# reilabs/gnark-whir

Hardware: AMD Instinct MI355X
Metric: Groth16 proofs/sec for WHIR-verifier circuit (2^20 poly); G1 MSM pts/sec (higher is better)
Workload: dtype u32x8 Montgomery (BN254 Fr/Fp, exact modular integers)

## Files before the change

### gnark-whir_amd/csrc/ntt.hip

```cpp
#include "ctx.h"
#include "ntt_wave.cuh"
#include "msm2_core.cuh"
#include <cstring>
#include <cstdlib>

struct NttState {
    u32 log_n = 0xffffffffu;
    Fr *small_f = nullptr, *small_i = nullptr, *tw64k_f = nullptr, *tw64k_i = nullptr;
    Fr *tw_lo_f = nullptr, *tw_hi_f = nullptr, *tw_lo_i = nullptr, *tw_hi_i = nullptr;
    Fr *g_lo = nullptr, *g_hi = nullptr, *gi_lo = nullptr, *gi_hi = nullptr, *ninv = nullptr;
    Fr *g_hi_n = nullptr, *gi_hi_nd = nullptr;
    Fr *ninv_den = nullptr;
    u32 tw_h = 0;
    Fr *d_tw_inv = nullptr, *d_tw_fwd = nullptr, *d_sc_fwd = nullptr, *d_sc_inv = nullptr;
    u32 d_log_n = 0xffffffffu, d_log_r0 = 0, d_npass = 0;
    u32 direct_min_log_n = 12;
    u32 log_e = 9, max_contig = 9, max_strided = 7, threads = 256;
    u32 lds_floor = 0;
    u32 plan_set = 0;
    u32 wave_stages = 1;
    u32 fuse_pair = 1;
    u32 fuse_triple = 1;
    u32 fuse_last = 1;
};
static NttKnobs knobs_for(const struct NttState *st, u32 log_n);
static NttState *state_of(mi_ctx *ctx) {
    static_assert(sizeof(NttState) <= 384, "NttState lives in ctx->ntt_state");
    return reinterpret_cast<NttState *>(ctx->ntt_state);
}

template <int CC> __global__ void k_ntt_contig_last_sub_count(Fr *A, const Fr *Cin, NttPass pa, NttTables ta, NttPass pc, NttTables tc, Msm2Shape zs, u32 *C1);
typedef void (*LastSubCountKernel)(Fr *, const Fr *, NttPass, NttTables, NttPass, NttTables, Msm2Shape, u32 *);
static const LastSubCountKernel k_last_sub_count[6] = {
    k_ntt_contig_last_sub_count<17>, k_ntt_contig_last_sub_count<18>, k_ntt_contig_last_sub_count<19>,
    k_ntt_contig_last_sub_count<20>, k_ntt_contig_last_sub_count<21>, k_ntt_contig_last_sub_count<22>};
bool mi_ntt_set_knob(mi_ctx *ctx, const char *name, int64_t value) {
    if (!std::strcmp(name, "ntt_lds_floor_kb") && value >= 0 && value <= 160) { state_of(ctx)->lds_floor = (u32)value * 1024u; return true; }
    return false;
}
void mi_ntt_state_free(mi_ctx *ctx) {
    NttState *st = state_of(ctx);
    Fr **all[] = {&st->small_f, &st->small_i, &st->tw64k_f, &st->tw64k_i, &st->g_hi_n, &st->gi_hi_nd, &st->tw_lo_f, &st->tw_hi_f, &st->tw_lo_i, &st->tw_hi_i,
                  &st->g_lo, &st->g_hi, &st->gi_lo, &st->gi_hi, &st->ninv, &st->ninv_den, &st->d_tw_inv, &st->d_tw_fwd, &st->d_sc_fwd, &st->d_sc_inv};
    for (Fr **p : all) if (*p) { (void)hipFree(*p); *p = nullptr; }
}

void mi_ntt_state_trim(mi_ctx *ctx) {
    mi_ntt_state_free(ctx);
    NttState *st = state_of(ctx);
    st->log_n = 0xffffffffu; st->d_log_n = 0xffffffffu; st->d_log_r0 = 0; st->d_npass = 0;
}
size_t mi_ntt_table_bytes(mi_ctx *ctx) {
    const NttState *st = state_of(ctx);
    size_t b = 0;
    if (st->small_f) b += (size_t)(2 * 2048 + 2 * 65536) * sizeof(Fr);
    if (st->log_n != 0xffffffffu) {
        const size_t nlo = (size_t)1 << st->tw_h, nhi = (size_t)1 << (st->log_n - st->tw_h);
        b += (4 * nlo + 6 * nhi + 2) * sizeof(Fr);
    }
    for (const Fr *p : {st->d_tw_inv, st->d_tw_fwd, st->d_sc_fwd, st->d_sc_inv}) if (p) b += sizeof(Fr) << st->d_log_n;
    return b;
}

static NttKnobs knobs_for(const NttState *st, u32 log_n) {
    if (st->plan_set) return NttKnobs{st->log_e, st->max_contig, st->max_strided};
    if (log_n == 24) return NttKnobs{10, 8, 8};
    if (log_n >= 25) return NttKnobs{10, 10, 8};
    return NttKnobs{st->log_e, st->max_contig, st->max_strided};
}

__global__ void k_pow_table(Fr *out, u32 count, Fr base, Fr c, u32 shift) {
    u32 j = blockIdx.x * blockDim.x + threadIdx.x;
    if (j >= count) return;
    u64 e = (u64)j << shift;
    Fr acc = c, b = base;
    while (e) {
        if (e & 1) acc = acc * b;
        b = fe_sqr(b);
        e >>= 1;
    }
    out[j] = acc;
}

__global__ void __launch_bounds__(1024) k_ntt_pass(Fr *dst, const Fr *src, NttPass p, NttTables t) {
    extern __shared__ U4 lds[];
    const u64 tile = blockIdx.x;
    ntt_tile_load(p, t, src, tile, threadIdx.x, blockDim.x, lds);
    __syncthreads();
    for (u32 s = 0; s < p.log_r; s++) {
        ntt_tile_stage(p, t, s, threadIdx.x, blockDim.x, lds);
        __syncthreads();
    }
    ntt_tile_store(p, t, dst, tile, threadIdx.x, blockDim.x, lds);
}

#ifndef MI_NTT_WAVES_PER_EU
#define MI_NTT_WAVES_PER_EU 1
#endif
__global__ void __launch_bounds__(256, MI_NTT_WAVES_PER_EU) k_ntt_pass_wave(Fr *dst, const Fr *src, NttPass p, NttTables t) {
    extern __shared__ U4 lds[];
    const u64 tile = blockIdx.x;
    const u32 PL = ntt_plane_slots(p);
    ntt_tile_load(p, t, src, tile, threadIdx.x, blockDim.x, lds);
    __syncthreads();
    if (!p.dit)
        for (u32 s = 0; s + 7 < p.log_r; s++) {
            ntt_tile_stage(p, t, s, threadIdx.x, blockDim.x, lds);
            __syncthreads();
        }
    const u32 lane = threadIdx.x & 63, wave = threadIdx.x >> 6, nwaves = blockDim.x >> 6;
    const u32 nsub = 1u << (p.log_r + p.log_c - 7);
    for (u32 sb = wave; sb < nsub; sb += nwaves) {
        const u32 col = sb & ((1u << p.log_c) - 1), base = (sb >> p.log_c) << 7;
        u32 ra, rb, wa, wb;
        if (!p.dit) { ra = base + lane; rb = ra + 64; wa = base + 2 * lane; wb = wa + 1; }
        else { ra = base + 2 * lane; rb = ra + 1; wa = base + lane; wb = wa + 64; }
        Fr x0 = lds_get(lds, PL, ntt_lds_slot(p, ra, col)), x1 = lds_get(lds, PL, ntt_lds_slot(p, rb, col));
        wave_ntt128(x0, x1, lane, p.dit != 0, t.small);
        lds_put(lds, PL, ntt_lds_slot(p, wa, col), x0);
        lds_put(lds, PL, ntt_lds_slot(p, wb, col), x1);
    }
    __syncthreads();
    if (p.dit)
        for (u32 s = 7; s < p.log_r; s++) {
            ntt_tile_stage(p, t, s, threadIdx.x, blockDim.x, lds);
            __syncthreads();
        }
    ntt_tile_store(p, t, dst, tile, threadIdx.x, blockDim.x, lds);
}

__global__ void __launch_bounds__(256) k_ntt_contig_pair(Fr *data, NttPass pi, NttTables ti, NttPass pf, NttTables tf) {
    extern __shared__ U4 lds[];
    const u64 tile = blockIdx.x;
    const u32 PL = ntt_plane_slots(pi);
    ntt_tile_load(pi, ti, data, tile, threadIdx.x, blockDim.x, lds);
    __syncthreads();
    for (u32 s = 0; s + 7 < pi.log_r; s++) {
        ntt_tile_stage(pi, ti, s, threadIdx.x, blockDim.x, lds);
        __syncthreads();
    }
    const u32 lane = threadIdx.x & 63, wave = threadIdx.x >> 6, nwaves = blockDim.x >> 6;
    const u32 nsub = 1u << (pi.log_r + pi.log_c - 7);
    for (u32 sb = wave; sb < nsub; sb += nwaves) {
        const u32 col = sb & ((1u << pi.log_c) - 1), base = (sb >> pi.log_c) << 7;
        Fr x0 = lds_get(lds, PL, ntt_lds_slot(pi, base + lane, col)), x1 = lds_get(lds, PL, ntt_lds_slot(pi, base + lane + 64, col));
        wave_ntt128(x0, x1, lane, false, ti.small);
        const u32 r0 = base + 2 * lane, r1 = r0 + 1;
        Fr f;
        if (ntt_edge_factor(pi, ti, r0, ntt_global_index(pi, tile, r0, col), 1, f)) x0 = fe_mul_lazy(x0, f);
        if (ntt_edge_factor(pf, tf, r0, ntt_global_index(pf, tile, r0, col), 0, f)) x0 = fe_mul_lazy(x0, f);
        if (ntt_edge_factor(pi, ti, r1, ntt_global_index(pi, tile, r1, col), 1, f)) x1 = fe_mul_lazy(x1, f);
        if (ntt_edge_factor(pf, tf, r1, ntt_global_index(pf, tile, r1, col), 0, f)) x1 = fe_mul_lazy(x1, f);
        wave_ntt128(x0, x1, lane, true, tf.small);
        lds_put(lds, PL, ntt_lds_slot(pf, base + lane, col), x0);
        lds_put(lds, PL, ntt_lds_slot(pf, base + lane + 64, col), x1);
    }
    __syncthreads();
    for (u32 s = 7; s < pf.log_r; s++) {
        ntt_tile_stage(pf, tf, s, threadIdx.x, blockDim.x, lds);
        __syncthreads();
    }
    ntt_tile_store(pf, tf, data, tile, threadIdx.x, blockDim.x, lds);
}

__global__ void __launch_bounds__(512) k_ntt_strided_triple(Fr *a, const Fr *b, NttPass pc, NttTables tc, NttPass pl, NttTables tl) {
    extern __shared__ U4 lds[];
    const u64 tile = blockIdx.x;
    const u32 PL = ntt_plane_slots(pc);
    const u32 lane = threadIdx.x & 63, sb = threadIdx.x >> 6;
    const u32 col = sb & ((1u << pc.log_c) - 1), base = (sb >> pc.log_c) << 7;
    const u32 s0 = ntt_lds_slot(pc, base + 2 * lane, col), s1 = ntt_lds_slot(pc, base + 2 * lane + 1, col);
    ntt_tile_load(pc, tc, a, tile, threadIdx.x, blockDim.x, lds);
    __syncthreads();
    Fr a0 = lds_get(lds, PL, s0), a1 = lds_get(lds, PL, s1);
    wave_ntt128(a0, a1, lane, true, tc.small);
    __syncthreads();
    ntt_tile_load(pc, tc, b, tile, threadIdx.x, blockDim.x, lds);
    __syncthreads();
    Fr x0 = lds_get(lds, PL, s0), x1 = lds_get(lds, PL, s1);
    wave_ntt128(x0, x1, lane, true, tc.small);
    x0 = ntt_mul_lazy2(x0, a0); x1 = ntt_mul_lazy2(x1, a1);
    wave_ntt128(x0, x1, lane, false, tl.small);
    __syncthreads();
    lds_put(lds, PL, ntt_lds_slot(pl, base + 2 * lane, col), x0);
    lds_put(lds, PL, ntt_lds_slot(pl, base + 2 * lane + 1, col), x1);
    __syncthreads();
    ntt_tile_store(pl, tl, a, tile, threadIdx.x, blockDim.x, lds);
}
__global__ void __launch_bounds__(256) k_ntt_strided_triple8(Fr *a, const Fr *b, NttPass pc, NttTables tc, NttPass pl, NttTables tl) {
    extern __shared__ U4 lds[];
    const u64 tile = blockIdx.x;
    const u32 PL = ntt_plane_slots(pc);
    const u32 lane = threadIdx.x & 63, wave = threadIdx.x >> 6, nwaves = blockDim.x >> 6;
    const u32 C = 1u << pc.log_c, nsub = 2u << pc.log_c;
    const u32 nb = C >> 1;
    Fr keep[4];
    auto reg_stages = [&](const NttPass &p, bool dit, const Fr *small) {
        for (u32 sbk = wave; sbk < nsub; sbk += nwaves) {
            const u32 col = sbk & (C - 1), base = (sbk >> p.log_c) << 7;
            u32 ra, rb, wa, wb;
            if (!dit) { ra = base + lane; rb = ra + 64; wa = base + 2 * lane; wb = wa + 1; }
            else { ra = base + 2 * lane; rb = ra + 1; wa = base + lane; wb = wa + 64; }
            Fr x0 = lds_get(lds, PL, ntt_lds_slot(p, ra, col)), x1 = lds_get(lds, PL, ntt_lds_slot(p, rb, col));
            wave_ntt128(x0, x1, lane, dit, small);
            lds_put(lds, PL, ntt_lds_slot(p, wa, col), x0);
            lds_put(lds, PL, ntt_lds_slot(p, wb, col), x1);
        }
    };
    ntt_tile_load(pc, tc, a, tile, threadIdx.x, blockDim.x, lds);
    __syncthreads();
    reg_stages(pc, true, tc.small);
    __syncthreads();
#pragma unroll
    for (u32 k = 0; k < 2; k++) {
        if (k >= nb) break;
        const u32 bf = threadIdx.x + 256 * k, col = bf & (C - 1), j = bf >> pc.log_c;
        Fr x = lds_get(lds, PL, ntt_lds_slot(pc, j, col));
        Fr y = lds_get(lds, PL, ntt_lds_slot(pc, j + 128, col));
        ntt_bfly_dit(x, y, j ? &tc.small[j << 4] : nullptr);
        keep[2 * k] = x; keep[2 * k + 1] = y;
    }
    __syncthreads();
    ntt_tile_load(pc, tc, b, tile, threadIdx.x, blockDim.x, lds);
    __syncthreads();
    reg_stages(pc, true, tc.small);
    __syncthreads();
#pragma unroll
    for (u32 k = 0; k < 2; k++) {
        if (k >= nb) break;
        const u32 bf = threadIdx.x + 256 * k, col = bf & (C - 1), j = bf >> pc.log_c;
        Fr x = lds_get(lds, PL, ntt_lds_slot(pc, j, col));
        Fr y = lds_get(lds, PL, ntt_lds_slot(pc, j + 128, col));
        ntt_bfly_dit(x, y, j ? &tc.small[j << 4] : nullptr);
        Fr p0 = ntt_mul_lazy2(x, keep[2 * k]), p1 = ntt_mul_lazy2(y, keep[2 * k + 1]);
        ntt_bfly_dif(p0, p1, j ? &tl.small[j << 4] : nullptr);
        lds_put(lds, PL, ntt_lds_slot(pl, j, col), p0);
        lds_put(lds, PL, ntt_lds_slot(pl, j + 128, col), p1);
    }
    __syncthreads();
    reg_stages(pl, false, tl.small);
    __syncthreads();
    ntt_tile_store(pl, tl, a, tile, threadIdx.x, blockDim.x, lds);
}

__device__ __forceinline__ void ntt_wave_pass_to_lds(const NttPass &p, const NttTables &t, const Fr *src, u64 tile, U4 *lds) {
    const u32 PL = ntt_plane_slots(p);
    ntt_tile_load(p, t, src, tile, threadIdx.x, blockDim.x, lds);
    __syncthreads();
    for (u32 s = 0; s + 7 < p.log_r; s++) {
        ntt_tile_stage(p, t, s, threadIdx.x, blockDim.x, lds);
        __syncthreads();
    }
    const u32 lane = threadIdx.x & 63, wave = threadIdx.x >> 6, nwaves = blockDim.x >> 6;
    const u32 nsub = 1u << (p.log_r + p.log_c - 7);
    for (u32 sb = wave; sb < nsub; sb += nwaves) {
        const u32 col = sb & ((1u << p.log_c) - 1), base = (sb >> p.log_c) << 7;
        Fr x0 = lds_get(lds, PL, ntt_lds_slot(p, base + lane, col)), x1 = lds_get(lds, PL, ntt_lds_slot(p, base + lane + 64, col));
        wave_ntt128(x0, x1, lane, false, t.small);
        lds_put(lds, PL, ntt_lds_slot(p, base + 2 * lane, col), x0);
        lds_put(lds, PL, ntt_lds_slot(p, base + 2 * lane + 1, col), x1);
    }
    __syncthreads();
}
template <int CC>
__device__ __forceinline__ void ntt_contig_last_sub_body(Fr *A, const Fr *Cin, const NttPass &pa, const NttTables &ta, const NttPass &pc, const NttTables &tc,
                                                         const Msm2Shape &zs, u32 *C1) {
    extern __shared__ U4 lds[];
    const u64 tile = blockIdx.x;
    const u32 E = 1u << (pa.log_r + pa.log_c), PL = ntt_plane_slots(pa);
    u32 *cnt = reinterpret_cast<u32 *>(lds + 2 * PL);
    const u32 nsl = E / MSM2_SLICE;
    if (CC >= 0) for (u32 k = threadIdx.x; k < nsl * zs.ngroups; k += blockDim.x) cnt[k] = 0;
    Fr keep[4];
    ntt_wave_pass_to_lds(pc, tc, Cin, tile, lds);
#pragma unroll
    for (u32 k = 0; k < 4; k++) {
        const u32 e = threadIdx.x + k * blockDim.x;
        if (e >= E) break;
        const u32 rho = e & ((1u << pc.log_r) - 1), col = e >> pc.log_r;
        Fr v = lds_get(lds, PL, ntt_lds_slot(pc, rho, col)), f;
        if (ntt_edge_factor(pc, tc, rho, ntt_global_index(pc, tile, rho, col), 1, f)) v = fe_mul_lazy(v, f);
        keep[k] = v;
    }
    __syncthreads();
    ntt_wave_pass_to_lds(pa, ta, A, tile, lds);
#pragma unroll
    for (u32 k = 0; k < 4; k++) {
        const u32 e = threadIdx.x + k * blockDim.x;
        if (e >= E) break;
        const u32 rho = e & ((1u << pa.log_r) - 1), col = e >> pa.log_r;
        const u64 g = ntt_global_index(pa, tile, rho, col);
        Fr v = lds_get(lds, PL, ntt_lds_slot(pa, rho, col)), f;
        if (ntt_edge_factor(pa, ta, rho, g, 1, f)) v = fe_mul_lazy(v, f);
        const Fr hv = fe_canon(fe_sub_plus2p(fe_condsub_2p(v), fe_condsub_2p(keep[k])));
        A[g] = hv;
        if (CC >= 0 && g < zs.n) {
            Msm2Digits dg;
            dg.start(hv, true);
            msm2_count_one<(CC >= 0 ? (u32)CC : 0u)>(zs, dg, cnt + (e / MSM2_SLICE) * zs.ngroups);
        }
    }
    if (CC >= 0) {
        __syncthreads();
        const u32 s0 = (u32)tile * nsl;
        for (u32 k = threadIdx.x; k < nsl * zs.ngroups; k += blockDim.x) {
            const u32 j = k / zs.ngroups, gq = k % zs.ngroups;
            if (s0 + j < zs.nslices) C1[(size_t)gq * zs.nslices + s0 + j] = cnt[k];
        }
    }
}
__global__ void __launch_bounds__(256) k_ntt_contig_last_sub(Fr *A, const Fr *Cin, NttPass pa, NttTables ta, NttPass pc, NttTables tc) {
    ntt_contig_last_sub_body<-1>(A, Cin, pa, ta, pc, tc, Msm2Shape{}, nullptr);
}
template <int CC>
__global__ void __launch_bounds__(256) k_ntt_contig_last_sub_count(Fr *A, const Fr *Cin, NttPass pa, NttTables ta, NttPass pc, NttTables tc, Msm2Shape zs, u32 *C1) {
    ntt_contig_last_sub_body<CC>(A, Cin, pa, ta, pc, tc, zs, C1);
}
void mi_ntt_state_init(mi_ctx *ctx) {
    static_assert(sizeof(NttState) <= sizeof(ctx->ntt_state), "NttState lives in ctx->ntt_state");
    new (ctx->ntt_state) NttState();
    const void *const dynamic_lds[] = {(const void *)k_ntt_pass, (const void *)k_ntt_pass_wave, (const void *)k_ntt_contig_pair,
                                       (const void *)k_ntt_strided_triple, (const void *)k_ntt_strided_triple8, (const void *)k_ntt_contig_last_sub};
    for (const void *k : dynamic_lds) (void)hipFuncSetAttribute(k, hipFuncAttributeMaxDynamicSharedMemorySize, 160 * 1024);
    for (LastSubCountKernel k : k_last_sub_count) (void)hipFuncSetAttribute((const void *)k, hipFuncAttributeMaxDynamicSharedMemorySize, 160 * 1024);
}

__global__ void k_tw_layout(Fr *out, u32 log_n, u32 log_r, Fr w) {
    const u32 g = blockIdx.x * blockDim.x + threadIdx.x;
    if (g >= (1u << log_n)) return;
    const u32 log_s = log_n - log_r;
    u32 e = (g & ((1u << log_s) - 1)) * bitrev_u32(g >> log_s, log_r);
    Fr acc = Fr::one(), b = w;
    while (e) { if (e & 1) acc = acc * b; b = fe_sqr(b); e >>= 1; }
    out[g] = acc;
}
__global__ void k_sc_layout(Fr *out, u32 log_n, Fr base, Fr c) {
    const u32 i = blockIdx.x * blockDim.x + threadIdx.x;
    if (i >= (1u << log_n)) return;
    u32 e = bitrev_u32(i, log_n);
    Fr acc = c, b = base;
    while (e) { if (e & 1) acc = acc * b; b = fe_sqr(b); e >>= 1; }
    out[i] = acc;
}

static int32_t build_table(mi_ctx *ctx, Fr **slot, u32 count, const Fr &base, const Fr &c, u32 shift) {
    if (*slot) { MI_CHECK_HIP(ctx, hipFree(*slot)); *slot = nullptr; }
    MI_CHECK_HIP(ctx, hipMalloc((void **)slot, sizeof(Fr) * (count ? count : 1)));
    hipLaunchKernelGGL(k_pow_table, dim3((count + 127) / 128), dim3(128), 0, ctx->stream, *slot, count, base, c, shift);
    MI_CHECK_HIP(ctx, hipGetLastError());
    return MI_OK;
}

struct NttRoots { Fr w, wi, g, gi, ninv, den; };
static NttRoots ntt_roots(u32 log_n) {
    NttRoots r;
    r.w = fr_domain_generator(log_n); r.wi = fe_inv(r.w);
    r.g = fe_from_u32<FrParams>(5); r.gi = fe_inv(r.g);
    Fr nn = Fr::zero();
    nn.l[0] = (u32)(1u << log_n);
    r.ninv = fe_inv(fe_to_mont(nn));
    Fr gn = r.g;
    for (u32 k = 0; k < log_n; k++) gn = fe_sqr(gn);
    r.den = fe_inv(gn - Fr::one());
    return r;
}

static int32_t ensure_tables(mi_ctx *ctx, u32 log_n) {
    NttState *st = state_of(ctx);
    if (!st->small_f) {
        Fr w4096 = fr_domain_generator(12);
        MI_TRY(build_table(ctx, &st->small_f, 2048, w4096, Fr::one(), 0));
        MI_TRY(build_table(ctx, &st->small_i, 2048, fe_inv(w4096), Fr::one(), 0));
        Fr w64k = fr_domain_generator(16);
        MI_TRY(build_table(ctx, &st->tw64k_f, 65536, w64k, Fr::one(), 0));
        MI_TRY(build_table(ctx, &st->tw64k_i, 65536, fe_inv(w64k), Fr::one(), 0));
    }
    if (st->log_n == log_n) return MI_OK;
    const NttRoots r = ntt_roots(log_n);
    u32 h = (log_n + 1) / 2;
    u32 nlo = 1u << h, nhi = 1u << (log_n - h);
    st->tw_h = h;
    MI_TRY(build_table(ctx, &st->tw_lo_f, nlo, r.w, Fr::one(), 0));
    MI_TRY(build_table(ctx, &st->tw_hi_f, nhi, r.w, Fr::one(), h));
    MI_TRY(build_table(ctx, &st->tw_lo_i, nlo, r.wi, Fr::one(), 0));
    MI_TRY(build_table(ctx, &st->tw_hi_i, nhi, r.wi, Fr::one(), h));
    MI_TRY(build_table(ctx, &st->g_lo, nlo, r.g, Fr::one(), 0));
    MI_TRY(build_table(ctx, &st->g_hi, nhi, r.g, Fr::one(), h));
    MI_TRY(build_table(ctx, &st->gi_lo, nlo, r.gi, Fr::one(), 0));
    MI_TRY(build_table(ctx, &st->gi_hi, nhi, r.gi, r.ninv, h));
    MI_TRY(build_table(ctx, &st->ninv, 1, Fr::one(), r.ninv, 0));
    MI_TRY(build_table(ctx, &st->g_hi_n, nhi, r.g, r.ninv, h));
    MI_TRY(build_table(ctx, &st->gi_hi_nd, nhi, r.gi, r.ninv * r.den, h));
    MI_TRY(build_table(ctx, &st->ninv_den, 1, Fr::one(), r.ninv * r.den, 0));
    st->log_n = log_n;
    return MI_OK;
}

static int32_t ensure_direct(mi_ctx *ctx, u32 log_n) {
    NttState *st = state_of(ctx);
    const NttKnobs kn = knobs_for(st, log_n);
    const NttPlan pl = ntt_make_plan(log_n, kn.max_contig, kn.max_strided);
    if (st->d_log_n == log_n && st->d_log_r0 == pl.log_r[0] && st->d_npass == pl.n_pass) return MI_OK;
    Fr **four[] = {&st->d_tw_inv, &st->d_tw_fwd, &st->d_sc_fwd, &st->d_sc_inv};
    for (Fr **p : four) if (*p) { (void)hipFree(*p); *p = nullptr; }
    st->d_log_n = 0xffffffffu;
    if (log_n < st->direct_min_log_n) return MI_OK;
    const size_t bytes = sizeof(Fr) << log_n;
    for (Fr **p : four)
        if (hipMalloc((void **)p, bytes) != hipSuccess) {
            (void)hipGetLastError();
            for (Fr **q : four) if (*q) { (void)hipFree(*q); *q = nullptr; }
            return MI_OK;
        }
    const NttRoots r = ntt_roots(log_n);
    const unsigned blocks = (unsigned)(((size_t)1 << log_n) + 255) / 256;
    if (pl.n_pass > 1) {
        hipLaunchKernelGGL(k_tw_layout, dim3(blocks), dim3(256), 0, ctx->stream, st->d_tw_inv, log_n, pl.log_r[0], r.wi);
        hipLaunchKernelGGL(k_tw_layout, dim3(blocks), dim3(256), 0, ctx->stream, st->d_tw_fwd, log_n, pl.log_r[0], r.w);
    }
    hipLaunchKernelGGL(k_sc_layout, dim3(blocks), dim3(256), 0, ctx->stream, st->d_sc_fwd, log_n, r.g, r.ninv);
    hipLaunchKernelGGL(k_sc_layout, dim3(blocks), dim3(256), 0, ctx->stream, st->d_sc_inv, log_n, r.gi, r.ninv * r.den);
    MI_CHECK_HIP(ctx, hipGetLastError());
    st->d_log_n = log_n; st->d_log_r0 = pl.log_r[0]; st->d_npass = pl.n_pass;
    return MI_OK;
}

static_assert(NTT_INVERSE == MI_NTT_INVERSE && NTT_COSET == MI_NTT_COSET && NTT_DIT == MI_NTT_DIT, "ntt_tile.cuh names the public flags");
static NttTransform ntt_build(const NttState *st, u32 log_n, u32 flags, NttVariant variant, u32 n_valid) {
    return ntt_build_transform(log_n, flags, variant, knobs_for(st, log_n), st->wave_stages != 0, n_valid);
}
static int32_t ntt_bind(mi_ctx *ctx, NttTransform &tr, const Fr *load_mul = nullptr, const Fr *store_sub = nullptr) {
    const NttState *st = state_of(ctx);
    const bool inverse = tr.flags & NTT_INVERSE, coset = tr.flags & NTT_COSET;
    NttTables &t = tr.t;
    t.small = inverse ? st->small_i : st->small_f;
    t.tw_lo = inverse ? st->tw_lo_i : st->tw_lo_f;
    t.tw_hi = inverse ? st->tw_hi_i : st->tw_hi_f;
    t.tw_h = st->tw_h;
    t.tw_64k = inverse ? st->tw64k_i : st->tw64k_f;
    if (coset && !inverse) { t.sc_lo = st->g_lo; t.sc_hi = tr.variant == NTT_COSET_FWD_NINV ? st->g_hi_n : st->g_hi; }
    else if (coset && inverse) { t.sc_lo = st->gi_lo; t.sc_hi = tr.variant == NTT_COSET_INV_DEN ? st->gi_hi_nd : st->gi_hi; }
    else if (inverse && tr.variant != NTT_INV_UNSCALED) t.sc_lo = t.sc_hi = tr.variant == NTT_INV_DEN_NINV ? st->ninv_den : st->ninv;
    NttPass &first = tr.pass[0];
    if (load_mul && (first.scale == 1 || first.scale == 2 || first.dit)) MI_FAIL(ctx, MI_EINVAL, "internal: load_mul on a pass whose load side already has a factor");
    first.load_mul = load_mul;
    tr.pass[tr.n_pass - 1].store_sub = store_sub;
    if (tr.variant == NTT_PLAIN || st->d_log_n != tr.log_n || !st->d_sc_fwd) return MI_OK;
    for (u32 i = 0; i < tr.n_pass; i++) {
        NttPass &p = tr.pass[i];
        if (p.twiddle && p.log_r + p.log_s == tr.log_n) p.tw_direct = inverse ? st->d_tw_inv : st->d_tw_fwd;
        if (tr.variant == NTT_COSET_FWD_NINV && p.scale == 1) p.sc_direct = st->d_sc_fwd;
        if (tr.variant == NTT_COSET_INV_DEN && p.scale == 3) p.sc_direct = st->d_sc_inv;
    }
    return MI_OK;
}

static u32 ntt_tiles(const NttPass &p) { return 1u << (p.log_n - p.log_r - p.log_c); }
static size_t ntt_lds_bytes(const NttPass &p) { return (size_t)32 * ntt_plane_slots(p); }
static int32_t ntt_launched(mi_ctx *ctx) {
    MI_CHECK_HIP(ctx, hipGetLastError());
    ctx->stats.ntt_launches++;
    return MI_OK;
}
static int32_t launch_pass(mi_ctx *ctx, Fr *dst, const Fr *src, const NttPass &p, const NttTables &t) {
    const NttState *st = state_of(ctx);
    const bool wave = p.log_r >= 7 && st->wave_stages;
    size_t lds_bytes = ntt_lds_bytes(p);
    if (st->lds_floor > lds_bytes) lds_bytes = st->lds_floor;
    const u32 E = 1u << (p.log_r + p.log_c);
    u32 threads = E / 2 >= st->threads ? st->threads : (E / 2 >= 64 ? E / 2 : 64);
    if (wave && threads > 256) threads = 256;
    void (*const kernel)(Fr *, const Fr *, NttPass, NttTables) = wave ? k_ntt_pass_wave : k_ntt_pass;
    hipLaunchKernelGGL(kernel, dim3(ntt_tiles(p)), dim3(threads), lds_bytes, ctx->stream, dst, src, p, t);
    return ntt_launched(ctx);
}
static int32_t launch_contig_pair(mi_ctx *ctx, Fr *v, const NttPass &pi, const NttTables &ti, const NttPass &pf, const NttTables &tf) {
    hipLaunchKernelGGL(k_ntt_contig_pair, dim3(ntt_tiles(pi)), dim3(256), ntt_lds_bytes(pi), ctx->stream, v, pi, ti, pf, tf);
    return ntt_launched(ctx);
}
static int32_t launch_strided_triple(mi_ctx *ctx, Fr *a, const Fr *b, const NttPass &pc, const NttTables &tc, const NttPass &pl, const NttTables &tl) {
    const bool r7 = pc.log_r == 7;
    void (*const kernel)(Fr *, const Fr *, NttPass, NttTables, NttPass, NttTables) = r7 ? k_ntt_strided_triple : k_ntt_strided_triple8;
    hipLaunchKernelGGL(kernel, dim3(ntt_tiles(pc)), dim3(r7 ? 64u << pc.log_c : 256u), ntt_lds_bytes(pc), ctx->stream, a, b, pc, tc, pl, tl);
    return ntt_launched(ctx);
}
static int32_t launch_contig_last_sub(mi_ctx *ctx, Fr *A, const Fr *C, const NttPass &pa, const NttTables &ta, const NttPass &pc, const NttTables &tc) {
    const size_t n = (size_t)1 << pa.log_n;
    const u32 E = 1u << (pa.log_r + pa.log_c);
    size_t lds_bytes = ntt_lds_bytes(pa);
    Msm2Shape zs{};
    bool count = ctx->zhook.armed && ctx->zhook.C1;
    if (count) {
        std::memcpy(&zs, ctx->zhook.shape, sizeof(zs));
        const size_t with_counters = lds_bytes + (size_t)(E / MSM2_SLICE) * zs.ngroups * 4;
        count = E % MSM2_SLICE == 0 && E / MSM2_SLICE <= 4 && zs.n <= n && (u64)zs.nslices * MSM2_SLICE == n && zs.c >= 17 && zs.c <= 22 && !zs.wkeys &&
                with_counters <= 160 * 1024;
        if (count) lds_bytes = with_counters;
    }
    ctx->zhook.armed = false;
    if (count) {
        hipLaunchKernelGGL(k_last_sub_count[zs.c - 17], dim3(ntt_tiles(pa)), dim3(256), lds_bytes, ctx->stream, A, C, pa, ta, pc, tc, zs, ctx->zhook.C1);
        ctx->zhook.done = true; ctx->zhook.h = A;
        ctx->z_count_fused_launches++;
    } else {
        hipLaunchKernelGGL(k_ntt_contig_last_sub, dim3(ntt_tiles(pa)), dim3(256), lds_bytes, ctx->stream, A, C, pa, ta, pc, tc);
    }
    return ntt_launched(ctx);
}
static int32_t launch_passes(mi_ctx *ctx, const NttTransform &tr, Fr *dst, const Fr *src, u32 from, u32 to) {
    for (u32 i = from; i < to; i++) MI_TRY(launch_pass(ctx, dst, i == 0 ? src : dst, tr.pass[i], tr.t));
    return MI_OK;
}

int32_t mi_ntt_dev_impl(mi_ctx *ctx, mi_fr *inout_dev, uint32_t log_n, uint32_t flags) {
    MI_TRY(ensure_tables(ctx, log_n));
    NttTransform tr = ntt_build(state_of(ctx), log_n, flags, NTT_PLAIN, 1u << log_n);
    MI_TRY(ntt_bind(ctx, tr));
    MI_TRY(launch_passes(ctx, tr, (Fr *)inout_dev, (const Fr *)inout_dev, 0, tr.n_pass));
    ctx->stats.ntt_elems += (u64)1 << log_n;
    return MI_OK;
}

struct ComputeHPlan {
    NttTransform inv, cos, cinv, last;
    u32 pair, triple, last_sub;
};
static bool same_tile(const NttPass &p, const NttPass &q) {
    return p.log_r == q.log_r && p.log_s == q.log_s && p.log_c == q.log_c && p.lds_pad == q.lds_pad;
}
static int32_t compute_h_plan(mi_ctx *ctx, u32 log_n, u32 n_valid, const Fr *c_mul, const Fr *B, const Fr *C, ComputeHPlan &cp) {
    const NttState *st = state_of(ctx);
    cp.inv = ntt_build(st, log_n, NTT_INVERSE, NTT_INV_UNSCALED, n_valid);
    cp.cos = ntt_build(st, log_n, NTT_DIT | NTT_COSET, NTT_COSET_FWD_NINV, 1u << log_n);
// ... 130 lines not shown
```

### gnark-whir_amd/csrc/ntt_tile.cuh

```cuda
#pragma once
#include "field.cuh"

struct alignas(16) U4 { u32 x, y, z, w; };

struct NttTables {
    const Fr *small;
    const Fr *tw_lo;
    const Fr *tw_hi;
    const Fr *sc_lo;
    const Fr *sc_hi;
    const Fr *tw_64k;
    u32 tw_h;
};

struct NttPass {
    u32 log_n;
    u32 log_r;
    u32 log_s;
    u32 log_c;
    u32 dit;
    u32 twiddle;
    u32 scale;
    u32 n_valid;
    u32 lds_pad;
    const Fr *tw_direct;
    const Fr *sc_direct;
    const Fr *load_mul;
    const Fr *store_sub;
    u32 canon;
};

MI_HD void ntt_bfly_dif(Fr &x0, Fr &x1, const Fr *w) {
    const Fr u = fe_condsub_2p(fe_add_nored(x0, x1));
    const Fr t = fe_sub_plus2p(x0, x1);
    x1 = w ? fe_mul_lazy(t, *w) : fe_condsub_2p(t);
    x0 = u;
}
MI_HD void ntt_bfly_dit(Fr &x0, Fr &x1, const Fr *w) {
    const Fr a = fe_condsub_2p(x0);
    const Fr t = w ? fe_mul_lazy(x1, *w) : fe_condsub_2p(x1);
    x0 = fe_add_nored(a, t);
    x1 = fe_sub_plus2p(a, t);
}
MI_HD Fr ntt_mul_lazy2(const Fr &x, const Fr &y) { return fe_mul_lazy(fe_condsub_2p(x), fe_condsub_2p(y)); }

MI_HD u32 bitrev_u32(u32 x, u32 bits) {
#if defined(__HIPCC__)
    return bits ? (__builtin_bitreverse32(x) >> (32 - bits)) : 0u;
#else
    u32 r = 0;
    for (u32 k = 0; k < bits; k++) { r = (r << 1) | (x & 1); x >>= 1; }
    return r;
#endif
}
MI_HD Fr pow_from_tables(const Fr *lo, const Fr *hi, u32 h, u32 e) {
    return lo[e & ((1u << h) - 1)] * hi[e >> h];
}

MI_HD u64 ntt_global_index(const NttPass &p, u64 tile, u32 rho, u32 col) {
    if (p.log_s == 0) return ((tile << p.log_c) + col) * ((u64)1 << p.log_r) + rho;
    u64 tiles_per_block = (u64)1 << (p.log_s - p.log_c);
    u64 hi = tile / tiles_per_block, lo0 = (tile % tiles_per_block) << p.log_c;
    return (hi << (p.log_r + p.log_s)) + ((u64)rho << p.log_s) + lo0 + col;
}
MI_HD u32 ntt_lds_slot(const NttPass &p, u32 rho, u32 col) {
    return p.log_s == 0 ? (col << p.log_r) + rho : rho * ((1u << p.log_c) + p.lds_pad) + col;
}
MI_HD u32 ntt_plane_slots(const NttPass &p) {
    return p.log_s == 0 ? 1u << (p.log_r + p.log_c) : ((1u << p.log_c) + p.lds_pad) << p.log_r;
}
MI_HD void lds_put(U4 *lds, u32 plane_elems, u32 slot, const Fr &v) {
    lds[slot] = U4{v.l[0], v.l[1], v.l[2], v.l[3]};
    lds[plane_elems + slot] = U4{v.l[4], v.l[5], v.l[6], v.l[7]};
}
MI_HD Fr lds_get(const U4 *lds, u32 plane_elems, u32 slot) {
    U4 a = lds[slot], b = lds[plane_elems + slot];
    Fr v;
    v.l[0] = a.x; v.l[1] = a.y; v.l[2] = a.z; v.l[3] = a.w;
    v.l[4] = b.x; v.l[5] = b.y; v.l[6] = b.z; v.l[7] = b.w;
    return v;
}
MI_HD bool ntt_edge_factor(const NttPass &p, const NttTables &t, u32 rho, u64 g, u32 phase, Fr &f) {
    const bool sc = phase == 0 ? (p.scale == 1 || p.scale == 2) : p.scale >= 3;
    const bool tw = p.twiddle && (phase == 0) == (p.dit != 0);
    const Fr *lo, *hi;
    u32 e;
    if (sc) {
        if (p.scale == 5) { f = t.sc_hi[0]; return true; }
        if (p.sc_direct) { f = p.sc_direct[g]; return true; }
        e = (p.scale == 1 || p.scale == 3) ? bitrev_u32((u32)g, p.log_n) : (u32)g;
        lo = t.sc_lo; hi = t.sc_hi;
    } else if (tw) {
        const u32 log_m = p.log_r + p.log_s;
        if (p.tw_direct) { f = p.tw_direct[g & (((u64)1 << log_m) - 1)]; return true; }
        const u32 x = (u32)(g & (((u64)1 << p.log_s) - 1)) * bitrev_u32(rho, p.log_r);
        if (t.tw_64k && log_m <= 16) { f = t.tw_64k[x << (16 - log_m)]; return true; }
        e = x << (p.log_n - log_m);
        lo = t.tw_lo; hi = t.tw_hi;
    } else if (phase == 0 && p.load_mul) {
        if (g >= p.n_valid) return false;
        f = p.load_mul[g];
        return true;
    } else {
        return false;
    }
    f = pow_from_tables(lo, hi, t.tw_h, e);
    return true;
}

MI_HD void ntt_tile_load(const NttPass &p, const NttTables &t, const Fr *data, u64 tile, u32 tid, u32 nthr, U4 *lds) {
    const u32 E = 1u << (p.log_r + p.log_c);
    for (u32 e = tid; e < E; e += nthr) {
        u32 rho, col;
        if (p.log_s == 0) { rho = e & ((1u << p.log_r) - 1); col = e >> p.log_r; }
        else { col = e & ((1u << p.log_c) - 1); rho = e >> p.log_c; }
        u64 g = ntt_global_index(p, tile, rho, col);
        Fr v = g < p.n_valid ? data[g] : Fr::zero(), f;
        if (ntt_edge_factor(p, t, rho, g, 0, f)) v = p.load_mul ? ntt_mul_lazy2(v, f) : fe_mul_lazy(v, f);
        lds_put(lds, ntt_plane_slots(p), ntt_lds_slot(p, rho, col), v);
    }
}
MI_HD void ntt_tile_stage(const NttPass &p, const NttTables &t, u32 stage, u32 tid, u32 nthr, U4 *lds) {
    const u32 E = 1u << (p.log_r + p.log_c);
    const u32 log_d = p.dit ? stage : (p.log_r - 1 - stage);
    const u32 d = 1u << log_d;
    for (u32 b = tid; b < E / 2; b += nthr) {
        u32 col, q;
        if (p.log_s == 0) { q = b & ((1u << (p.log_r - 1)) - 1); col = b >> (p.log_r - 1); }
        else { col = b & ((1u << p.log_c) - 1); q = b >> p.log_c; }
        u32 j = q & (d - 1);
        u32 r0 = ((q >> log_d) << (log_d + 1)) + j;
        u32 r1 = r0 + d;
        u32 s0 = ntt_lds_slot(p, r0, col), s1 = ntt_lds_slot(p, r1, col);
        const u32 PL = ntt_plane_slots(p);
        Fr x = lds_get(lds, PL, s0), y = lds_get(lds, PL, s1);
        const Fr *w = j ? &t.small[j << (11 - log_d)] : nullptr;
        if (p.dit) ntt_bfly_dit(x, y, w); else ntt_bfly_dif(x, y, w);
        lds_put(lds, PL, s0, x);
        lds_put(lds, PL, s1, y);
    }
}
MI_HD void ntt_tile_store(const NttPass &p, const NttTables &t, Fr *data, u64 tile, u32 tid, u32 nthr, const U4 *lds) {
    const u32 E = 1u << (p.log_r + p.log_c);
    for (u32 e = tid; e < E; e += nthr) {
        u32 rho, col;
        if (p.log_s == 0) { rho = e & ((1u << p.log_r) - 1); col = e >> p.log_r; }
        else { col = e & ((1u << p.log_c) - 1); rho = e >> p.log_c; }
        u64 g = ntt_global_index(p, tile, rho, col);
        Fr v = lds_get(lds, ntt_plane_slots(p), ntt_lds_slot(p, rho, col)), f;
        if (ntt_edge_factor(p, t, rho, g, 1, f)) v = fe_mul_lazy(v, f);
        if (p.store_sub) v = fe_sub_plus2p(fe_condsub_2p(v), fe_condsub_2p(p.store_sub[g]));
        if (p.canon) v = fe_canon(v);
        data[g] = v;
    }
}

struct NttPlan {
    u32 n_pass;
    u32 log_r[8];
};
MI_HD NttPlan ntt_make_plan(u32 log_n, u32 max_contig, u32 max_strided) {
    NttPlan pl;
    pl.n_pass = 0;
    if (log_n <= max_contig) { pl.n_pass = 1; pl.log_r[0] = log_n; return pl; }
    u32 rest = log_n - max_contig;
    u32 ns = (rest + max_strided - 1) / max_strided;
    for (u32 i = 0; i < ns; i++) {
        u32 r = rest / (ns - i);
        pl.log_r[pl.n_pass++] = r;
        rest -= r;
    }
    pl.log_r[pl.n_pass++] = max_contig;
    return pl;
}

enum : u32 { NTT_INVERSE = 1, NTT_COSET = 2, NTT_DIT = 4 };
enum NttVariant : u32 {
    NTT_PLAIN = 0,
    NTT_INV_UNSCALED = 1,
    NTT_COSET_FWD_NINV = 2,
    NTT_COSET_INV_DEN = 3,
    NTT_INV_DEN_NINV = 4,
};
struct NttKnobs { u32 log_e, max_contig, max_strided; };
struct NttTransform {
    u32 log_n, flags;
    NttVariant variant;
    u32 n_pass;
    NttPass pass[8];
    NttTables t;
};
inline NttTransform ntt_build_transform(u32 log_n, u32 flags, NttVariant variant, NttKnobs kn, bool wave_stages, u32 n_valid) {
    const bool inverse = flags & NTT_INVERSE, coset = flags & NTT_COSET, dit = flags & NTT_DIT;
    u32 load_scale = 0, store_scale = 0;
    if (coset && !inverse) load_scale = dit ? 1 : 2;
    else if (coset && inverse) store_scale = dit ? 4 : 3;
    else if (inverse && variant != NTT_INV_UNSCALED) store_scale = 5;
    const NttPlan pl = ntt_make_plan(log_n, kn.max_contig, kn.max_strided);
    u32 log_s[8];
    for (u32 i = 0, acc = log_n; i < pl.n_pass; i++) { acc -= pl.log_r[i]; log_s[i] = acc; }
    NttTransform tr{};
    tr.log_n = log_n; tr.flags = flags; tr.variant = variant; tr.n_pass = pl.n_pass;
    for (u32 step = 0; step < pl.n_pass; step++) {
        const u32 i = dit ? pl.n_pass - 1 - step : step;
        const bool first = step == 0, last = step == pl.n_pass - 1;
        NttPass &p = tr.pass[step];
        p.log_n = log_n; p.log_r = pl.log_r[i]; p.log_s = log_s[i];
        const u32 room = kn.log_e > p.log_r ? kn.log_e - p.log_r : 0;
        const u32 avail = p.log_s == 0 ? log_n - p.log_r : p.log_s;
        p.log_c = room < avail ? room : avail;
        p.dit = dit ? 1 : 0;
        p.twiddle = p.log_s != 0;
        p.scale = first && load_scale ? load_scale : last ? store_scale : 0;
        p.n_valid = first ? n_valid : (1u << log_n);
        p.lds_pad = wave_stages && p.log_r >= 7 && p.log_s != 0 ? 1 : 0;
        p.canon = last && (variant == NTT_PLAIN || variant == NTT_COSET_INV_DEN);
    }
    return tr;
}
// ... 1 lines not shown
```

### gnark-whir_amd/csrc/ntt_wave.cuh

```cuda
#pragma once
#include "ntt_tile.cuh"

MI_D Fr wave_trade(const Fr &v, u32 src_lane) {
    Fr r;
#pragma unroll
    for (int i = 0; i < 8; i++) r.l[i] = (u32)__builtin_amdgcn_ds_bpermute((int)(src_lane << 2), (int)v.l[i]);
    return r;
}
MI_D void wave_select_trade(Fr &x0, Fr &x1, u32 lane, u32 m) {
    const bool hi = (lane & m) != 0;
    Fr send;
#pragma unroll
    for (int i = 0; i < 8; i++) send.l[i] = hi ? x0.l[i] : x1.l[i];
    const Fr recv = wave_trade(send, lane ^ m);
#pragma unroll
    for (int i = 0; i < 8; i++) { x0.l[i] = hi ? recv.l[i] : x0.l[i]; x1.l[i] = hi ? x1.l[i] : recv.l[i]; }
}
MI_D void wave_ntt128(Fr &x0, Fr &x1, u32 lane, bool dit, const Fr *small) {
    if (!dit) {
#pragma unroll 1
        for (int log_d = 6; log_d >= 0; log_d--) {
            const u32 d = 1u << log_d;
            if (log_d < 6) wave_select_trade(x0, x1, lane, d);
            ntt_bfly_dif(x0, x1, log_d ? &small[(lane & (d - 1)) << (11 - log_d)] : nullptr);
        }
    } else {
#pragma unroll 1
        for (int log_d = 0; log_d <= 6; log_d++) {
            const u32 d = 1u << log_d;
            if (log_d) wave_select_trade(x0, x1, lane, d >> 1);
            ntt_bfly_dit(x0, x1, log_d ? &small[(lane & (d - 1)) << (11 - log_d)] : nullptr);
        }
    }
}
```

Baseline: 33.69.

## Fold inter-pass twiddles into per-stage butterfly twiddle tables for strided NTT passes

Adds per-strided-pass precomputed twiddle tables laid out per column so each butterfly stage uses a combined twiddle. This removes the separate inter-pass twiddle multiply at load/store. The wave NTT prefetches the next stage's twiddle from global memory. The cost is extra table memory of size 2^(log_r+log_s) per pass and scattered global twiddle loads instead of small LDS/L1-resident tables.

Measured after the change: 34.37 (median of 6 runs). 1.02x the previous value.

```diff
diff --git a/gnark-whir_amd/csrc/ntt.hip b/gnark-whir_amd/csrc/ntt.hip
--- a/gnark-whir_amd/csrc/ntt.hip
+++ b/gnark-whir_amd/csrc/ntt.hip
@@ -14,6 +14,10 @@
     u32 tw_h = 0;
     Fr *d_tw_inv = nullptr, *d_tw_fwd = nullptr, *d_sc_fwd = nullptr, *d_sc_inv = nullptr;
     u32 d_log_n = 0xffffffffu, d_log_r0 = 0, d_npass = 0;
+    Fr *s_tw_inv[3] = {nullptr, nullptr, nullptr}, *s_tw_fwd[3] = {nullptr, nullptr, nullptr};
+    u32 s_log_r[3] = {0, 0, 0}, s_log_s[3] = {0, 0, 0}, s_n = 0;
+    u32 stage_tw = 1;
+    u32 d_radices = 0, d_stage_tw = 0;
     u32 direct_min_log_n = 12;
     u32 log_e = 9, max_contig = 9, max_strided = 7, threads = 256;
     u32 lds_floor = 0;
@@ -36,13 +40,20 @@
     k_ntt_contig_last_sub_count<20>, k_ntt_contig_last_sub_count<21>, k_ntt_contig_last_sub_count<22>};
 bool mi_ntt_set_knob(mi_ctx *ctx, const char *name, int64_t value) {
     if (!std::strcmp(name, "ntt_lds_floor_kb") && value >= 0 && value <= 160) { state_of(ctx)->lds_floor = (u32)value * 1024u; return true; }
+    if (!std::strcmp(name, "ntt_stage_twiddles") && (value == 0 || value == 1)) { state_of(ctx)->stage_tw = (u32)value; return true; }
     return false;
+}
+static void free_stage_tables(NttState *st) {
+    for (u32 k = 0; k < 3; k++)
+        for (Fr **p : {&st->s_tw_inv[k], &st->s_tw_fwd[k]}) if (*p) { (void)hipFree(*p); *p = nullptr; }
+    st->s_n = 0;
 }
 void mi_ntt_state_free(mi_ctx *ctx) {
     NttState *st = state_of(ctx);
     Fr **all[] = {&st->small_f, &st->small_i, &st->tw64k_f, &st->tw64k_i, &st->g_hi_n, &st->gi_hi_nd, &st->tw_lo_f, &st->tw_hi_f, &st->tw_lo_i, &st->tw_hi_i,
                   &st->g_lo, &st->g_hi, &st->gi_lo, &st->gi_hi, &st->ninv, &st->ninv_den, &st->d_tw_inv, &st->d_tw_fwd, &st->d_sc_fwd, &st->d_sc_inv};
     for (Fr **p : all) if (*p) { (void)hipFree(*p); *p = nullptr; }
+    free_stage_tables(st);
 }
 
 void mi_ntt_state_trim(mi_ctx *ctx) {
@@ -59,6 +70,7 @@
         b += (4 * nlo + 6 * nhi + 2) * sizeof(Fr);
     }
     for (const Fr *p : {st->d_tw_inv, st->d_tw_fwd, st->d_sc_fwd, st->d_sc_inv}) if (p) b += sizeof(Fr) << st->d_log_n;
+    for (u32 k = 0; k < st->s_n; k++) b += 2 * (sizeof(Fr) << (st->s_log_r[k] + st->s_log_s[k]));
     return b;
 }
 
@@ -88,7 +100,7 @@
     ntt_tile_load(p, t, src, tile, threadIdx.x, blockDim.x, lds);
     __syncthreads();
     for (u32 s = 0; s < p.log_r; s++) {
-        ntt_tile_stage(p, t, s, threadIdx.x, blockDim.x, lds);
+        ntt_tile_stage(p, t, s, threadIdx.x, blockDim.x, lds, tile);
         __syncthreads();
     }
     ntt_tile_store(p, t, dst, tile, threadIdx.x, blockDim.x, lds);
@@ -105,7 +117,7 @@
     __syncthreads();
     if (!p.dit)
         for (u32 s = 0; s + 7 < p.log_r; s++) {
-            ntt_tile_stage(p, t, s, threadIdx.x, blockDim.x, lds);
+            ntt_tile_stage(p, t, s, threadIdx.x, blockDim.x, lds, tile);
             __syncthreads();
         }
     const u32 lane = threadIdx.x & 63, wave = threadIdx.x >> 6, nwaves = blockDim.x >> 6;
@@ -116,14 +128,14 @@
         if (!p.dit) { ra = base + lane; rb = ra + 64; wa = base + 2 * lane; wb = wa + 1; }
         else { ra = base + 2 * lane; rb = ra + 1; wa = base + lane; wb = wa + 64; }
         Fr x0 = lds_get(lds, PL, ntt_lds_slot(p, ra, col)), x1 = lds_get(lds, PL, ntt_lds_slot(p, rb, col));
-        wave_ntt128(x0, x1, lane, p.dit != 0, t.small);
+        wave_ntt128(x0, x1, lane, p.dit != 0, t.small, ntt_stage_run(p, tile, col));
         lds_put(lds, PL, ntt_lds_slot(p, wa, col), x0);
         lds_put(lds, PL, ntt_lds_slot(p, wb, col), x1);
     }
     __syncthreads();
     if (p.dit)
         for (u32 s = 7; s < p.log_r; s++) {
-            ntt_tile_stage(p, t, s, threadIdx.x, blockDim.x, lds);
+            ntt_tile_stage(p, t, s, threadIdx.x, blockDim.x, lds, tile);
             __syncthreads();
         }
     ntt_tile_store(p, t, dst, tile, threadIdx.x, blockDim.x, lds);
@@ -170,17 +182,18 @@
     const u32 lane = threadIdx.x & 63, sb = threadIdx.x >> 6;
     const u32 col = sb & ((1u << pc.log_c) - 1), base = (sb >> pc.log_c) << 7;
     const u32 s0 = ntt_lds_slot(pc, base + 2 * lane, col), s1 = ntt_lds_slot(pc, base + 2 * lane + 1, col);
+    const Fr *const run_c = ntt_stage_run(pc, tile, col), *const run_l = ntt_stage_run(pl, tile, col);
     ntt_tile_load(pc, tc, a, tile, threadIdx.x, blockDim.x, lds);
     __syncthreads();
     Fr a0 = lds_get(lds, PL, s0), a1 = lds_get(lds, PL, s1);
-    wave_ntt128(a0, a1, lane, true, tc.small);
+    wave_ntt128(a0, a1, lane, true, tc.small, run_c);
     __syncthreads();
     ntt_tile_load(pc, tc, b, tile, threadIdx.x, blockDim.x, lds);
     __syncthreads();
     Fr x0 = lds_get(lds, PL, s0), x1 = lds_get(lds, PL, s1);
-    wave_ntt128(x0, x1, lane, true, tc.small);
+    wave_ntt128(x0, x1, lane, true, tc.small, run_c);
     x0 = ntt_mul_lazy2(x0, a0); x1 = ntt_mul_lazy2(x1, a1);
-    wave_ntt128(x0, x1, lane, false, tl.small);
+    wave_ntt128(x0, x1, lane, false, tl.small, run_l);
     __syncthreads();
     lds_put(lds, PL, ntt_lds_slot(pl, base + 2 * lane, col), x0);
     lds_put(lds, PL, ntt_lds_slot(pl, base + 2 * lane + 1, col), x1);
@@ -202,7 +215,7 @@
             if (!dit) { ra = base + lane; rb = ra + 64; wa = base + 2 * lane; wb = wa + 1; }
             else { ra = base + 2 * lane; rb = ra + 1; wa = base + lane; wb = wa + 64; }
             Fr x0 = lds_get(lds, PL, ntt_lds_slot(p, ra, col)), x1 = lds_get(lds, PL, ntt_lds_slot(p, rb, col));
-            wave_ntt128(x0, x1, lane, dit, small);
+            wave_ntt128(x0, x1, lane, dit, small, ntt_stage_run(p, tile, col));
             lds_put(lds, PL, ntt_lds_slot(p, wa, col), x0);
             lds_put(lds, PL, ntt_lds_slot(p, wb, col), x1);
         }
@@ -217,7 +230,8 @@
         const u32 bf = threadIdx.x + 256 * k, col = bf & (C - 1), j = bf >> pc.log_c;
         Fr x = lds_get(lds, PL, ntt_lds_slot(pc, j, col));
         Fr y = lds_get(lds, PL, ntt_lds_slot(pc, j + 128, col));
-        ntt_bfly_dit(x, y, j ? &tc.small[j << 4] : nullptr);
+        const Fr *run = ntt_stage_run(pc, tile, col);
+        ntt_bfly_dit(x, y, run ? &run[128 + j] : j ? &tc.small[j << 4] : nullptr);
         keep[2 * k] = x; keep[2 * k + 1] = y;
     }
     __syncthreads();
@@ -231,9 +245,10 @@
         const u32 bf = threadIdx.x + 256 * k, col = bf & (C - 1), j = bf >> pc.log_c;
         Fr x = lds_get(lds, PL, ntt_lds_slot(pc, j, col));
         Fr y = lds_get(lds, PL, ntt_lds_slot(pc, j + 128, col));
-        ntt_bfly_dit(x, y, j ? &tc.small[j << 4] : nullptr);
+        const Fr *run_c = ntt_stage_run(pc, tile, col), *run_l = ntt_stage_run(pl, tile, col);
+        ntt_bfly_dit(x, y, run_c ? &run_c[128 + j] : j ? &tc.small[j << 4] : nullptr);
         Fr p0 = ntt_mul_lazy2(x, keep[2 * k]), p1 = ntt_mul_lazy2(y, keep[2 * k + 1]);
-        ntt_bfly_dif(p0, p1, j ? &tl.small[j << 4] : nullptr);
+        ntt_bfly_dif(p0, p1, run_l ? &run_l[128 + j] : j ? &tl.small[j << 4] : nullptr);
         lds_put(lds, PL, ntt_lds_slot(pl, j, col), p0);
         lds_put(lds, PL, ntt_lds_slot(pl, j + 128, col), p1);
     }
@@ -334,6 +349,14 @@
     while (e) { if (e & 1) acc = acc * b; b = fe_sqr(b); e >>= 1; }
     out[g] = acc;
 }
+__global__ void k_tw_stage_layout(Fr *out, u32 log_n, u32 log_r, u32 log_s, Fr w) {
+    const u32 idx = blockIdx.x * blockDim.x + threadIdx.x;
+    if (idx >= (1u << (log_r + log_s))) return;
+    u32 e = ntt_stage_tw_exponent(log_n, log_r, log_s, idx);
+    Fr acc = Fr::one(), b = w;
+    while (e) { if (e & 1) acc = acc * b; b = fe_sqr(b); e >>= 1; }
+    out[idx] = acc;
+}
 __global__ void k_sc_layout(Fr *out, u32 log_n, Fr base, Fr c) {
     const u32 i = blockIdx.x * blockDim.x + threadIdx.x;
     if (i >= (1u << log_n)) return;
@@ -400,28 +423,51 @@
     NttState *st = state_of(ctx);
     const NttKnobs kn = knobs_for(st, log_n);
     const NttPlan pl = ntt_make_plan(log_n, kn.max_contig, kn.max_strided);
-    if (st->d_log_n == log_n && st->d_log_r0 == pl.log_r[0] && st->d_npass == pl.n_pass) return MI_OK;
+    u32 radices = 0;
+    for (u32 i = 0; i < pl.n_pass; i++) radices |= pl.log_r[i] << (4 * i);
+    if (st->d_log_n == log_n && st->d_log_r0 == pl.log_r[0] && st->d_npass == pl.n_pass && st->d_radices == radices && st->d_stage_tw == st->stage_tw) return MI_OK;
     Fr **four[] = {&st->d_tw_inv, &st->d_tw_fwd, &st->d_sc_fwd, &st->d_sc_inv};
     for (Fr **p : four) if (*p) { (void)hipFree(*p); *p = nullptr; }
+    free_stage_tables(st);
     st->d_log_n = 0xffffffffu;
     if (log_n < st->direct_min_log_n) return MI_OK;
+    const u32 n_strided = pl.n_pass - 1;
+    bool stage = st->stage_tw && n_strided >= 1 && n_strided <= 3;
+    for (u32 k = 0, log_s = log_n; stage && k < n_strided; k++) {
+        log_s -= pl.log_r[k];
+        st->s_log_r[k] = pl.log_r[k]; st->s_log_s[k] = log_s;
+        for (Fr **p : {&st->s_tw_inv[k], &st->s_tw_fwd[k]})
+            if (stage && hipMalloc((void **)p, sizeof(Fr) << (pl.log_r[k] + log_s)) != hipSuccess) { (void)hipGetLastError(); *p = nullptr; stage = false; }
+    }
+    if (!stage) free_stage_tables(st);
     const size_t bytes = sizeof(Fr) << log_n;
-    for (Fr **p : four)
+    for (Fr **p : four) {
+        if (stage && (p == &st->d_tw_inv || p == &st->d_tw_fwd)) continue;
         if (hipMalloc((void **)p, bytes) != hipSuccess) {
             (void)hipGetLastError();
+            *p = nullptr;
             for (Fr **q : four) if (*q) { (void)hipFree(*q); *q = nullptr; }
+            free_stage_tables(st);
             return MI_OK;
         }
+    }
     const NttRoots r = ntt_roots(log_n);
     const unsigned blocks = (unsigned)(((size_t)1 << log_n) + 255) / 256;
-    if (pl.n_pass > 1) {
+    if (stage) {
+        st->s_n = n_strided;
+        for (u32 k = 0; k < n_strided; k++) {
+            const unsigned sb = (unsigned)((((size_t)1 << (st->s_log_r[k] + st->s_log_s[k])) + 255) / 256);
+            hipLaunchKernelGGL(k_tw_stage_layout, dim3(sb), dim3(256), 0, ctx->stream, st->s_tw_inv[k], log_n, st->s_log_r[k], st->s_log_s[k], r.wi);
+            hipLaunchKernelGGL(k_tw_stage_layout, dim3(sb), dim3(256), 0, ctx->stream, st->s_tw_fwd[k], log_n, st->s_log_r[k], st->s_log_s[k], r.w);
+        }
+    } else if (pl.n_pass > 1) {
         hipLaunchKernelGGL(k_tw_layout, dim3(blocks), dim3(256), 0, ctx->stream, st->d_tw_inv, log_n, pl.log_r[0], r.wi);
         hipLaunchKernelGGL(k_tw_layout, dim3(blocks), dim3(256), 0, ctx->stream, st->d_tw_fwd, log_n, pl.log_r[0], r.w);
     }
     hipLaunchKernelGGL(k_sc_layout, dim3(blocks), dim3(256), 0, ctx->stream, st->d_sc_fwd, log_n, r.g, r.ninv);
     hipLaunchKernelGGL(k_sc_layout, dim3(blocks), dim3(256), 0, ctx->stream, st->d_sc_inv, log_n, r.gi, r.ninv * r.den);
     MI_CHECK_HIP(ctx, hipGetLastError());
-    st->d_log_n = log_n; st->d_log_r0 = pl.log_r[0]; st->d_npass = pl.n_pass;
+    st->d_log_n = log_n; st->d_log_r0 = pl.log_r[0]; st->d_npass = pl.n_pass; st->d_radices = radices; st->d_stage_tw = st->stage_tw;
     return MI_OK;
 }
 
@@ -448,7 +494,9 @@
     if (tr.variant == NTT_PLAIN || st->d_log_n != tr.log_n || !st->d_sc_fwd) return MI_OK;
     for (u32 i = 0; i < tr.n_pass; i++) {
         NttPass &p = tr.pass[i];
-        if (p.twiddle && p.log_r + p.log_s == tr.log_n) p.tw_direct = inverse ? st->d_tw_inv : st->d_tw_fwd;
+        for (u32 k = 0; p.twiddle && k < st->s_n; k++)
+            if (st->s_log_r[k] == p.log_r && st->s_log_s[k] == p.log_s) p.tw_stage = inverse ? st->s_tw_inv[k] : st->s_tw_fwd[k];
+        if (p.twiddle && !p.tw_stage && p.log_r + p.log_s == tr.log_n) p.tw_direct = inverse ? st->d_tw_inv : st->d_tw_fwd;
         if (tr.variant == NTT_COSET_FWD_NINV && p.scale == 1) p.sc_direct = st->d_sc_fwd;
         if (tr.variant == NTT_COSET_INV_DEN && p.scale == 3) p.sc_direct = st->d_sc_inv;
     }
diff --git a/gnark-whir_amd/csrc/ntt_tile.cuh b/gnark-whir_amd/csrc/ntt_tile.cuh
--- a/gnark-whir_amd/csrc/ntt_tile.cuh
+++ b/gnark-whir_amd/csrc/ntt_tile.cuh
@@ -28,7 +28,16 @@
     const Fr *load_mul;
     const Fr *store_sub;
     u32 canon;
-};
+    const Fr *tw_stage;
+};
+MI_HD u32 ntt_stage_tw_exponent(u32 log_n, u32 log_r, u32 log_s, u32 idx) {
+    const u32 k = idx & ((1u << log_r) - 1), lo = idx >> log_r;
+    if (!k) return 0;
+    u32 log_d = 0;
+    while ((2u << log_d) <= k) log_d++;
+    const u32 j = k - (1u << log_d);
+    return ((j << log_s) + lo) << (log_n - 1 - log_d - log_s);
+}
 
 MI_HD void ntt_bfly_dif(Fr &x0, Fr &x1, const Fr *w) {
     const Fr u = fe_condsub_2p(fe_add_nored(x0, x1));
@@ -80,9 +89,14 @@
     v.l[4] = b.x; v.l[5] = b.y; v.l[6] = b.z; v.l[7] = b.w;
     return v;
 }
+MI_HD const Fr *ntt_stage_run(const NttPass &p, u64 tile, u32 col) {
+    if (!p.tw_stage) return nullptr;
+    const u64 lo = ((tile & (((u64)1 << (p.log_s - p.log_c)) - 1)) << p.log_c) + col;
+    return p.tw_stage + (lo << p.log_r);
+}
 MI_HD bool ntt_edge_factor(const NttPass &p, const NttTables &t, u32 rho, u64 g, u32 phase, Fr &f) {
     const bool sc = phase == 0 ? (p.scale == 1 || p.scale == 2) : p.scale >= 3;
-    const bool tw = p.twiddle && (phase == 0) == (p.dit != 0);
+    const bool tw = p.twiddle && !p.tw_stage && (phase == 0) == (p.dit != 0);
     const Fr *lo, *hi;
     u32 e;
     if (sc) {
@@ -120,7 +134,7 @@
         lds_put(lds, ntt_plane_slots(p), ntt_lds_slot(p, rho, col), v);
     }
 }
-MI_HD void ntt_tile_stage(const NttPass &p, const NttTables &t, u32 stage, u32 tid, u32 nthr, U4 *lds) {
+MI_HD void ntt_tile_stage(const NttPass &p, const NttTables &t, u32 stage, u32 tid, u32 nthr, U4 *lds, u64 tile = 0) {
     const u32 E = 1u << (p.log_r + p.log_c);
     const u32 log_d = p.dit ? stage : (p.log_r - 1 - stage);
     const u32 d = 1u << log_d;
@@ -134,7 +148,8 @@
         u32 s0 = ntt_lds_slot(p, r0, col), s1 = ntt_lds_slot(p, r1, col);
         const u32 PL = ntt_plane_slots(p);
         Fr x = lds_get(lds, PL, s0), y = lds_get(lds, PL, s1);
-        const Fr *w = j ? &t.small[j << (11 - log_d)] : nullptr;
+        const Fr *run = ntt_stage_run(p, tile, col);
+        const Fr *w = run ? &run[d + j] : j ? &t.small[j << (11 - log_d)] : nullptr;
         if (p.dit) ntt_bfly_dit(x, y, w); else ntt_bfly_dif(x, y, w);
         lds_put(lds, PL, s0, x);
         lds_put(lds, PL, s1, y);
diff --git a/gnark-whir_amd/csrc/ntt_wave.cuh b/gnark-whir_amd/csrc/ntt_wave.cuh
--- a/gnark-whir_amd/csrc/ntt_wave.cuh
+++ b/gnark-whir_amd/csrc/ntt_wave.cuh
@@ -16,7 +16,33 @@
 #pragma unroll
     for (int i = 0; i < 8; i++) { x0.l[i] = hi ? recv.l[i] : x0.l[i]; x1.l[i] = hi ? x1.l[i] : recv.l[i]; }
 }
-MI_D void wave_ntt128(Fr &x0, Fr &x1, u32 lane, bool dit, const Fr *small) {
+MI_D void wave_ntt128_tw(Fr &x0, Fr &x1, u32 lane, bool dit, const Fr *run) {
+    if (!dit) {
+        Fr w = run[64 + lane];
+#pragma unroll 1
+        for (int log_d = 6; log_d >= 0; log_d--) {
+            const u32 d = 1u << log_d;
+            Fr wn = w;
+            if (log_d) wn = run[(d >> 1) + (lane & ((d >> 1) - 1))];
+            if (log_d < 6) wave_select_trade(x0, x1, lane, d);
+            ntt_bfly_dif(x0, x1, &w);
+            w = wn;
+        }
+    } else {
+        Fr w = run[1];
+#pragma unroll 1
+        for (int log_d = 0; log_d <= 6; log_d++) {
+            const u32 d = 1u << log_d;
+            Fr wn = w;
+            if (log_d < 6) wn = run[2 * d + (lane & (2 * d - 1))];
+            if (log_d) wave_select_trade(x0, x1, lane, d >> 1);
+            ntt_bfly_dit(x0, x1, &w);
+            w = wn;
+        }
+    }
+}
+MI_D void wave_ntt128(Fr &x0, Fr &x1, u32 lane, bool dit, const Fr *small, const Fr *run = nullptr) {
+    if (run) { wave_ntt128_tw(x0, x1, lane, dit, run); return; }
     if (!dit) {
 #pragma unroll 1
         for (int log_d = 6; log_d >= 0; log_d--) {
```
